# gabrielmittag/NISQA

Measured on AMD Instinct MI355X. Metric: clips/sec (10 s, 48 kHz), higher is better.
Workload: dtype bf16x6 (every GEMM -- CNN, projection, self-attention, pooling: fp32 operands as three exact bf16 terms, 6 MFMA products per term pair, f32 accumulate: all 24 operand mantissa bits; mel f32)

## Files before the change

nisqa_amd/csrc/cnn_bf16.hip:

```cpp
#include "common.hpp"
#include "layout.hpp"
#include <stdlib.h>
#include <atomic>
#include "conv_bf16.hpp"
#include "internal.hpp"
#include "../../include/nisqa_hip.h"
#define NQ_RING2 3
#define NQ_RING34 3

#define FB_RS1 48
#define FB_P1 (168 * FB_RS1)
#define FB_RS2 80
#define FB_P2 (60 * FB_RS2)
#define FB_RS3 144
#define FB_P3 (60 * FB_RS3)
#define FB_PS (72 * FB_RS3)
#define FB_PATCH(T) ((T) * FB_P1)
#define FB_PPLANE 1700
#define FB_ZADDR 2048u
#define FB_BASE 2176u
#define FB_WAVE(T) (((T) * (FB_P1 + FB_PPLANE) + 63u) / 64u * 64u)
#define FB_WGS(T) ((T) == 2 ? 2 : 1)
#define FB_LDS(T) (FB_BASE + 4 * FB_WAVE(T))
static_assert(FB_WAVE(2) == 19584 && FB_LDS(2) == 80512 && 2 * FB_LDS(2) <= 160 * 1024, "two terms: two workgroups (8 waves) per CU");
static_assert(FB_WAVE(3) == 29312 && FB_LDS(3) == 119424 && FB_LDS(3) <= 160 * 1024 && 2 * FB_LDS(3) > 160 * 1024, "three terms: one workgroup per CU");
#define FB_PLAN_OK(T) (FB_PATCH(T) + (T) * FB_PPLANE <= FB_WAVE(T) && (T) * FB_P3 <= FB_WAVE(T) && (T) * FB_PS <= 2 * FB_WAVE(T))
static_assert(FB_PLAN_OK(2) && FB_PLAN_OK(3), "LDS plan");

__device__ constexpr int bwin75_lo(int b) { return b == 0 ? 0 : b == 1 ? 1 : b == 2 ? 2 : b == 3 ? 4 : 5; }
__device__ constexpr int bwin75_hi(int b) { return b == 0 ? 2 : b == 1 ? 3 : b == 2 ? 5 : b == 3 ? 6 : 7; }
__device__ constexpr int bwin53_lo(int b) { return b == 0 ? 0 : b == 1 ? 1 : 3; }
__device__ constexpr int bwin53_hi(int b) { return b == 0 ? 2 : b == 1 ? 4 : 5; }

NQ_CLK_EXPORT(g_phase_clk, nisqa_debug_phase_clock)
NQ_CLK_EXPORT(g_phase_clk6, nisqa_debug_phase_clock6)

#define FB_TAB5 0u
#define FB_TAB6 1024u
NQ_DEV f32x2_t lds_ld64(unsigned a) { return *(NQ_AS3 const f32x2_t*)(a); }
template <int FMT>
NQ_DEV float epi_fmt(float v, float c, float t) {
    return FMT == NQ_FMT_BF16X3 || FMT == NQ_FMT_BF16X6 ? fmaxf(v + t, 0.f) : fmaxf(fmaf(v, c, t), 0.f);
}

template <int FMT, int CIN, int MT, int NT, int W, int RS, int PLANE, bool APF, int RING>
NQ_DEV void fb_conv_k(f32x16 (&acc)[MT][NT], __amdgpu_buffer_rsrc_t wrs, int wbyte, unsigned lane16, const unsigned (&base)[MT],
                      const unsigned (&m9)[MT], conv_k_ring<FMT == NQ_FMT_BF16X6 ? 3 : 2, NT, 3>& ring) {
    if constexpr (FMT == NQ_FMT_BF16X6) conv_k_terms_ring<3, CIN, MT, NT, W, RS, PLANE, FB_ZADDR, 3, true, true>(acc, wrs, wbyte, lane16, base, m9, ring);
    else conv_k_bf16<CIN, MT, NT, W, RS, PLANE, FB_ZADDR, APF, RING, FMT>(acc, wrs, wbyte, lane16, base, m9);
}

template <int FMT, bool SEGX, bool P3>
NQ_DEV void cnn_front_split_body(
    const float* __restrict__ mel_tm, const int32_t* __restrict__ frame_off,
    const int32_t* __restrict__ tok_off, const int32_t* __restrict__ n_wins,
    const float* __restrict__ clip_floor, int n_clips, int seg_hop,
    const float* __restrict__ cw, const unsigned short* __restrict__ wb, float* __restrict__ p3,
    float* __restrict__ feat, const float* __restrict__ seg_x, int seg_L,
    const uint32_t* __restrict__ clip_max_enc, float top_db) {
    extern __shared__ __attribute__((aligned(16))) char smem[];
    constexpr bool X6 = FMT == NQ_FMT_BF16X6, F16 = FMT == NQ_FMT_F16X3 || FMT == NQ_FMT_F16X4;
    constexpr int T = X6 ? 3 : 2;
    constexpr bool T16_3 = X6 && (NQ_T16 & 1), T16_4 = X6 && (NQ_T16 & 2);
    static_assert(!P3 || FMT == NQ_FMT_BF16X3, "the fp32 copy of the pooled conv4 tensor is a bf16x3 debug output");
    constexpr int W1_ = X6 ? CNNX_W1 : CNNB_W1, W2_ = X6 ? CNNX_W2 : CNNB_W2, W3_ = X6 ? CNNX_W3 : CNNB_W3, W4_ = X6 ? CNNX_W4 : CNNB_W4,
                  W5_ = X6 ? CNNX_W5 : CNNB_W5, W6_ = X6 ? CNNX_W6 : CNNB_W6, WU16_ = X6 ? CNNX_U16S : CNNB_U16S;
    const int* __restrict__ meta_i = (const int*)(wb + CNNH_META);
    const float* __restrict__ meta_f = (const float*)(wb + CNNH_META);
    float dummy_mx = 0.f;
    NQ_STAMP_BEGIN();
    const int lane = threadIdx.x & 63;
    const int wave = __builtin_amdgcn_readfirstlane(threadIdx.x >> 6);
    const int p0 = blockIdx.x * 4;
    const int b = __builtin_amdgcn_readfirstlane(find_segment_wave(tok_off, n_clips, p0, lane));
    const int k0 = p0 - tok_off[b];
    const int nvalid = min(4, n_wins[b] - k0);
    if (nvalid <= 0) return;
    const bool valid = wave < nvalid;
    const int p = p0 + wave, k = k0 + wave;
    const unsigned R = FB_BASE + wave * FB_WAVE(T);
    const unsigned lane16 = lane * 16;
    const __amdgpu_buffer_rsrc_t wrs = __builtin_amdgcn_make_buffer_rsrc((void*)wb, 0, WU16_ * 2, 0x00020000);
    NQ_STAMP(0);

    const float fl = SEGX ? -3.0e38f : clip_max_enc ? dec_ordered(clip_max_enc[b]) - top_db : clip_floor[b];
    const float* src = SEGX ? seg_x + ((size_t)b * seg_L + k) * 720
                            : mel_tm + (size_t)(frame_off[b] + k * seg_hop) * 48;
    float vraw[12];
#pragma unroll
    for (int q = 0; q < 12; ++q) {
        const int i0 = lane + 64 * q;
        vraw[q] = (valid && (q < 11 || lane < 16)) ? src[i0] : 0.f;
    }
    const float tn1 = cw[CNN_T1 + (lane & 15)], tn2 = cw[CNN_T2 + (lane & 31)];
    const float tn3[2] = {cw[CNN_T3 + (lane & 31)], cw[CNN_T3 + 32 + (lane & 31)]};
    const float tn4[2] = {cw[CNN_T4 + (lane & 31)], cw[CNN_T4 + 32 + (lane & 31)]};
    const float tn5 = cw[CNN_T5 + 16 * wave + (lane & 15)], tn6 = cw[CNN_T6 + 16 * wave + (lane & 15)];
    float vin[12];
#pragma unroll
    for (int q = 0; q < 12; ++q) vin[q] = !valid ? 0.f : SEGX ? vraw[q] : fmaxf(vraw[q], fl);
    int e_in = 0;
    float m_in = 0.f;
    float s0 = 1.f;
    if (F16) {
        float mr = 0.f;
#pragma unroll
        for (int q = 0; q < 12; ++q) mr = fmaxf(mr, __builtin_fabsf(vin[q]));
        m_in = wave_max_nonneg(mr);
        e_in = f16_scale_exp(m_in);
        s0 = pow2_f32(e_in);
    }
    {
        const unsigned pb = R + FB_PATCH(T);
        constexpr int NZ = (T * FB_PPLANE + 15) / 16;
#pragma unroll
        for (int it = 0; it < (NZ + 63) / 64; ++it)
            if (64 * it + 64 <= NZ || lane < NZ - 64 * it) lds_st128(pb + (lane + 64 * it) * 16, f32x4{0.f, 0.f, 0.f, 0.f});
        if (lane < 32) ((unsigned*)(smem + FB_ZADDR))[lane] = 0u;
        __builtin_amdgcn_wave_barrier();
        if (!SEGX) {
            unsigned ob[3];
#pragma unroll
            for (int u = 0; u < 3; ++u) {
                const int e = lane + 16 * u, j0 = e >= 48 ? 1 : 0, m = e - 48 * j0;
                ob[u] = pb + ((j0 + 1) * 50 + m + 1) * 2;
            }
#pragma unroll
            for (int q = 0; q < 12; q += 2) {
                const float v0 = vin[q] * s0, v1 = vin[q + 1] * s0;
                lds_store_pair_fmt<FMT>(ob[q % 3] + (q + q / 3) * 100, ob[(q + 1) % 3] + (q + 1 + (q + 1) / 3) * 100, FB_PPLANE, v0, v1,
                                               dummy_mx, true, q + 1 < 11 || lane < 16);
            }
        } else {
#pragma unroll
            for (int q = 0; q < 12; ++q) {
                const int i0 = lane + 64 * q;
                const int m = i0 / 15, j = i0 - 15 * m;
                if (i0 < 720) lds_store_one_fmt<FMT>(pb + ((j + 1) * 50 + (m + 1)) * 2, FB_PPLANE, vin[q] * s0, dummy_mx);
            }
        }
    }
    __builtin_amdgcn_wave_barrier();
    NQ_STAMP(1);

    const int i = lane & 31, hfi = (i >> 2) & 1, qi = (i & 3) + 4 * (i >> 3);
    const int n = lane & 31, hf = lane >> 5, h = lane >> 5;

    conv_k_ring<T, 1, 3> ring2;
    if constexpr (X6) conv_k_preload(ring2, wrs, W2_ * 2, lane16);
    {
        f32x4 w1[1][T];
#pragma unroll
        for (int t = 0; t < T; ++t) w1[0][t] = wfrag_load(wrs, lane16, (W1_ + t * 512) * 2);
        float tn = tn1, c1 = 1.f, ms1 = 0.f;
        int e1 = 0;
        if (F16) {
            e1 = f16_scale_exp(fmaf(m_in, meta_f[8], meta_f[16]));
            c1 = pow2_f32(e1 - e_in - meta_i[0]);
            tn = tn1 * pow2_f32(e1);
        }
        const int xq = min(qi, 14);
        unsigned rd_a = R + FB_PATCH(T) + ((xq + (h ? 2 : 0)) * 50 + 24 * hfi) * 2;
        unsigned rd_b = R + FB_PATCH(T) + ((xq + (h ? 2 : 1)) * 50 + 24 * hfi) * 2;
        const bool is_b = (n & 16) != 0;
        const unsigned mb = is_b ? ~0u : 0u;
        unsigned wr = R + (12 * hf * 7) * FB_RS1 + (n & 15) * 2 + (is_b ? FB_RS1 : 0);
        for (int g2 = 0; g2 < 6; ++g2) {
            f32x16 acc[2][1];
            f32x4 xa[2][T];
#pragma unroll
            for (int tt = 0; tt < 2; ++tt)
#pragma unroll
                for (int t = 0; t < T; ++t) {
                    const unsigned pa = rd_a + 4 * tt + t * FB_PPLANE, pq = rd_b + 4 * tt + t * FB_PPLANE;
                    xa[tt][t] = f32x4{__uint_as_float(lds_ld32(pa)), __uint_as_float(lds_ld32(pa + 4)),
                                      __uint_as_float(lds_ld32(pq)), __uint_as_float(lds_ld32(pq + 4))};
                }
            acc[0][0] = zero16();
            acc[1][0] = zero16();
            if constexpr (X6) {
                mma_terms<T, 2, 1>(acc, xa, w1);
            } else {
                const f32x4 (&w)[T] = w1[0];
                if (FMT == NQ_FMT_F16X4) { acc[0][0] = mfma32_fmt<FMT>(xa[0][1], w[1], acc[0][0]); acc[1][0] = mfma32_fmt<FMT>(xa[1][1], w[1], acc[1][0]); }
                acc[0][0] = mfma32_fmt<FMT>(xa[0][1], w[0], acc[0][0]); acc[1][0] = mfma32_fmt<FMT>(xa[1][1], w[0], acc[1][0]);
                acc[0][0] = mfma32_fmt<FMT>(xa[0][0], w[1], acc[0][0]); acc[1][0] = mfma32_fmt<FMT>(xa[1][0], w[1], acc[1][0]);
                acc[0][0] = mfma32_fmt<FMT>(xa[0][0], w[0], acc[0][0]); acc[1][0] = mfma32_fmt<FMT>(xa[1][0], w[0], acc[1][0]);
            }
            unsigned r[14];
#pragma unroll
            for (int v = 0; v < 14; ++v) {
                const int tt = v / 7, bb = v - 7 * tt;
                const float mx = fmaxf(fmaxf(acc[tt][0][2 * bb], acc[tt][0][2 * bb + 1]), acc[tt][0][2 * bb + 2]);
                r[v] = __float_as_uint(epi_fmt<FMT>(mx, c1, tn));
            }
            unsigned got[7];
#pragma unroll
            for (int kk = 0; kk < 7; ++kk)
                got[kk] = (unsigned)__builtin_amdgcn_ds_swizzle((int)((r[2 * kk] & mb) | (r[2 * kk + 1] & ~mb)), 0x401F);
            float fin[7];
#pragma unroll
            for (int kk = 0; kk < 7; ++kk) {
                const unsigned own = (r[2 * kk + 1] & mb) | (r[2 * kk] & ~mb);
                fin[kk] = __uint_as_float(max(own, got[kk]));
            }
#pragma unroll
            for (int kk = 0; kk < 6; kk += 2) lds_store_pair_fmt<FMT>(wr + 2 * kk * FB_RS1, wr + 2 * (kk + 1) * FB_RS1, FB_P1, fin[kk], fin[kk + 1], ms1);
            lds_store_one_fmt<FMT>(wr + 12 * FB_RS1, FB_P1, fin[6], ms1);
            rd_a += 8; rd_b += 8;
            wr += 14 * FB_RS1;
        }
        if (F16) { m_in = wave_max_nonneg(ms1) * pow2_f32(-e1); e_in = e1; }
    }

    NQ_STAMP(2);
    conv_k_ring<T, 2, 3> ring34;
    conv_kt_ring<T, 4, NQ_RINGT> ringt;
    const unsigned lanew = conv_kt_lane<T, 4>(lane);
    const int c16 = lane & 15, q4 = lane >> 4;
    f32x4 tnt[4];
    {
        f32x16 acc[6][1];
        unsigned base[6], m9[6];
#pragma unroll
        for (int t = 0; t < 6; ++t) {
            acc[t][0] = zero16();
            const int u = 16 * t + qi;
            const int gl = u / 14, w = u % 14, yy = w / 7;
            const int py = 2 * (6 * hfi + gl) + yy, px = w - 7 * yy;
            m9[t] = tap_mask(u < 84, py, px, 24, 7);
            base[t] = R + ((py - 1) * 7 + (px - 1)) * FB_RS1 + (h << 4);
        }
        fb_conv_k<FMT, 16, 6, 1, 7, FB_RS1, FB_P1, false, NQ_RING2>(acc, wrs, W2_ * 2, lane16, base, m9, ring2);
        NQ_STAMP(3);
        if constexpr (T16_3) {
            conv_kt_preload(ringt, wrs, W3_ * 2, lanew);
#pragma unroll
            for (int mt = 0; mt < 4; ++mt) tnt[mt] = *(const f32x4*)(cw + CNN_T3 + 16 * mt + 4 * q4);
            __builtin_amdgcn_sched_barrier(0);
        } else if constexpr (X6) {
            conv_k_preload(ring34, wrs, W3_ * 2, lane16);
            __builtin_amdgcn_sched_barrier(0);
        }
        float tn = tn2, c2 = 1.f, ms2 = 0.f;
        int e2 = 0;
        if (F16) {
            e2 = f16_scale_exp(fmaf(m_in, meta_f[9], meta_f[17]));
            c2 = pow2_f32(e2 - e_in - meta_i[1]);
            tn = tn2 * pow2_f32(e2);
        }
        const unsigned wr = R + (6 * hf * 5) * FB_RS2 + n * 2;
#pragma unroll
        for (int k2 = 0; k2 < 30; k2 += 2) {
            float pv[2];
#pragma unroll
            for (int e = 0; e < 2; ++e) {
                const int gl = (k2 + e) / 5, bb = (k2 + e) % 5;
                float mx = -3.0e38f;
#pragma unroll
                for (int yy = 0; yy < 2; ++yy)
#pragma unroll
                    for (int x = bwin75_lo(bb); x < bwin75_hi(bb); ++x) {
                        const int u = 14 * gl + 7 * yy + x;
                        mx = fmaxf(mx, acc[u >> 4][0][u & 15]);
                    }
                pv[e] = epi_fmt<FMT>(mx, c2, tn);
            }
            lds_store_pair_fmt<FMT>(wr + k2 * FB_RS2, wr + (k2 + 1) * FB_RS2, FB_P2, pv[0], pv[1], ms2);
        }
        if (F16) { m_in = wave_max_nonneg(ms2) * pow2_f32(-e2); e_in = e2; }
    }

    NQ_STAMP(4);
    unsigned base34[2], m34[2];
#pragma unroll
    for (int t = 0; t < 2; ++t) {
        const int u = 16 * t + qi;
        const int gl = u / 10, w = u % 10, yy = w / 5;
        const int py = 2 * (3 * hfi + gl) + yy, px = w - 5 * yy;
        m34[t] = tap_mask(u < 30, py, px, 12, 5);
        base34[t] = (py - 1) * 5 + (px - 1);
    }

    if constexpr (T16_3) {
        f32x4 acc[4][4];
        unsigned base[4], m9[4];
#pragma unroll
        for (int nt = 0; nt < 4; ++nt) {
#pragma unroll
            for (int mt = 0; mt < 4; ++mt) acc[mt][nt] = f32x4{0.f, 0.f, 0.f, 0.f};
            const int pix = 16 * nt + c16, py = pix / 5, px = pix - 5 * py;
            m9[nt] = tap_mask(pix < 60, py, px, 12, 5);
            base[nt] = R + (pix - 6) * FB_RS2 + (q4 << 4);
        }
        conv_kt_terms_ring<3, 32, 4, 4, 5, FB_RS2, FB_P2, FB_ZADDR, NQ_RINGT>(acc, wrs, W3_ * 2, lanew, base, m9, ringt);
        NQ_STAMP(5);
        const f32x4 tn[4] = {tnt[0], tnt[1], tnt[2], tnt[3]};
        if constexpr (T16_4) {
            conv_kt_preload(ringt, wrs, W4_ * 2, lanew);
#pragma unroll
            for (int mt = 0; mt < 4; ++mt) tnt[mt] = *(const f32x4*)(cw + CNN_T4 + 16 * mt + 4 * q4);
        } else conv_k_preload(ring34, wrs, W4_ * 2, lane16);
        __builtin_amdgcn_sched_barrier(0);
        const unsigned wr = R + c16 * FB_RS3 + q4 * 8;
#pragma unroll
        for (int nt = 0; nt < 4; ++nt)
            if (nt < 3 || c16 < 12) {
#pragma unroll
                for (int mt = 0; mt < 4; ++mt) {
                    f32x4 v;
#pragma unroll
                    for (int r = 0; r < 4; ++r) v[r] = fmaxf(acc[mt][nt][r] + tn[mt][r], 0.f);
                    lds_store_terms4<3>(wr + 16 * nt * FB_RS3 + 32 * mt, FB_P3, v);
                }
            }
    } else {
        f32x16 acc[2][2];
        unsigned base[2];
#pragma unroll
        for (int t = 0; t < 2; ++t) {
#pragma unroll
            for (int nt = 0; nt < 2; ++nt) acc[t][nt] = zero16();
            base[t] = R + base34[t] * FB_RS2 + (h << 4);
        }
        fb_conv_k<FMT, 32, 2, 2, 5, FB_RS2, FB_P2, true, NQ_RING34>(acc, wrs, W3_ * 2, lane16, base, m34, ring34);
        NQ_STAMP(5);
        if constexpr (T16_4) {
            conv_kt_preload(ringt, wrs, W4_ * 2, lanew);
#pragma unroll
            for (int mt = 0; mt < 4; ++mt) tnt[mt] = *(const f32x4*)(cw + CNN_T4 + 16 * mt + 4 * q4);
            __builtin_amdgcn_sched_barrier(0);
        } else if constexpr (X6) {
            conv_k_preload(ring34, wrs, W4_ * 2, lane16);
            __builtin_amdgcn_sched_barrier(0);
        }
        float tn[2] = {tn3[0], tn3[1]}, c3 = 1.f, ms3 = 0.f;
        int e3 = 0;
        if (F16) {
            e3 = f16_scale_exp(fmaf(m_in, meta_f[10], meta_f[18]));
            c3 = pow2_f32(e3 - e_in - meta_i[2]);
            tn[0] *= pow2_f32(e3);
            tn[1] *= pow2_f32(e3);
        }
        const unsigned wr = R + (6 * hf * 5) * FB_RS3 + n * 2;
#pragma unroll
        for (int nt = 0; nt < 2; ++nt)
#pragma unroll
            for (int t = 0; t < 2; ++t)
#pragma unroll
                for (int r = 0; r < 16; r += 2) {
                    const int u = 16 * t + r;
                    if (u < 30)
                        lds_store_pair_fmt<FMT>(wr + u * FB_RS3 + 64 * nt, wr + (u + 1) * FB_RS3 + 64 * nt, FB_P3,
                                                epi_fmt<FMT>(acc[t][nt][r], c3, tn[nt]), epi_fmt<FMT>(acc[t][nt][r + 1], c3, tn[nt]), ms3);
                }
        if (F16) { m_in = wave_max_nonneg(ms3) * pow2_f32(-e3); e_in = e3; }
    }

    NQ_STAMP(6);
    const unsigned S4 = FB_BASE;
    const unsigned S5 = FB_BASE + 2 * FB_WAVE(T);
    const int w5b = __builtin_amdgcn_readfirstlane((W5_ + wave * (18 * T * 512)) * 2);
    const int w6b = __builtin_amdgcn_readfirstlane((W6_ + wave * (18 * T * 512)) * 2);
    f32x4 b5[4][T], b6[8][T];
    if constexpr (T16_4) {
        f32x4 acc[4][4];
        unsigned base[4], m9[4];
        const int j5 = c16 / 5, role = c16 - 5 * j5;
        const int glc = 2 * j5 + (role >= 3 ? 1 : 0);
#pragma unroll
        for (int nt = 0; nt < 4; ++nt) {
#pragma unroll
            for (int mt = 0; mt < 4; ++mt) acc[mt][nt] = f32x4{0.f, 0.f, 0.f, 0.f};
            const int yy = nt & 1, hi = nt >> 1;
            const int gl = role == 2 ? 2 * j5 + hi : glc;
            const int px = role == 2 ? 2 : role == 0 ? hi : role == 3 ? 1 - hi : 3 + hi, py = 2 * gl + yy;
            m9[nt] = tap_mask(c16 < 15, py, px, 12, 5);
            base[nt] = R + (py * 5 + px - 6) * FB_RS3 + (q4 << 4);
        }
        conv_kt_terms_ring<3, 64, 4, 4, 5, FB_RS3, FB_P3, FB_ZADDR, NQ_RINGT>(acc, wrs, W4_ * 2, lanew, base, m9, ringt);
        NQ_STAMP(7);
#pragma unroll
        for (int g = 0; g < 3; ++g)
#pragma unroll
            for (int q = 0; q < T; ++q) b5[g][q] = wfrag_load(wrs, lane16, w5b + (g * T + q) * 1024);
        f32x4 w02[4], w1[4];
#pragma unroll
        for (int mt = 0; mt < 4; ++mt)
#pragma unroll
            for (int r = 0; r < 4; ++r) {
                const float m01 = __builtin_elementwise_maximum(acc[mt][0][r], acc[mt][1][r]), m23 = __builtin_elementwise_maximum(acc[mt][2][r], acc[mt][3][r]);
                const int i01 = (int)__float_as_uint(m01), i23 = (int)__float_as_uint(m23);
                const float lf = __uint_as_float((unsigned)__builtin_amdgcn_update_dpp(i23, i23, 0x111, 0xf, 0xf, false));
                const float rt = __uint_as_float((unsigned)__builtin_amdgcn_update_dpp(i01, i01, 0x101, 0xf, 0xf, false));
                w02[mt][r] = fmaxf(__builtin_elementwise_maximum(m01, m23) + tnt[mt][r], 0.f);
                w1[mt][r] = fmaxf(__builtin_elementwise_maximum(__builtin_elementwise_maximum(m01, lf), rt) + tnt[mt][r], 0.f);
            }
        __syncthreads();
        const unsigned wr = S4 + (18 * wave + 3 * glc) * FB_RS3 + q4 * 8;
        if (c16 < 15 && role != 2) {
            const unsigned a = wr + (role == 1 || role == 4 ? 2 * FB_RS3 : 0);
#pragma unroll
            for (int mt = 0; mt < 4; ++mt) lds_store_terms4<3>(a + 32 * mt, FB_PS, w02[mt]);
        }
        if (c16 < 15 && (role == 1 || role == 3)) {
#pragma unroll
            for (int mt = 0; mt < 4; ++mt) lds_store_terms4<3>(wr + FB_RS3 + 32 * mt, FB_PS, w1[mt]);
        }
    } else {
        f32x16 acc[2][2];
        unsigned base[2];
#pragma unroll
        for (int t = 0; t < 2; ++t) {
#pragma unroll
            for (int nt = 0; nt < 2; ++nt) acc[t][nt] = zero16();
            base[t] = R + base34[t] * FB_RS3 + (h << 4);
        }
        fb_conv_k<FMT, 64, 2, 2, 5, FB_RS3, FB_P3, true, NQ_RING34>(acc, wrs, W4_ * 2, lane16, base, m34, ring34);
        NQ_STAMP(7);
        float tn[2] = {tn4[0], tn4[1]}, c4 = 1.f, ms4 = 0.f;
        int e4 = 0;
        if (F16) {
            e4 = f16_scale_exp(fmaf(m_in, meta_f[11], meta_f[19]));
            c4 = pow2_f32(e4 - e_in - meta_i[3]);
            tn[0] *= pow2_f32(e4);
            tn[1] *= pow2_f32(e4);
        }
#pragma unroll
        for (int g = 0; g < 3; ++g)
#pragma unroll
            for (int q = 0; q < T; ++q) b5[g][q] = wfrag_load(wrs, lane16, w5b + (g * T + q) * 1024);
        __syncthreads();
        const unsigned wr = S4 + (18 * wave + 9 * hf) * FB_RS3 + n * 2;
        float* dst = P3 ? p3 + (size_t)p * (18 * 64) : nullptr;
#pragma unroll
        for (int gl = 0; gl < 3; ++gl)
#pragma unroll
            for (int bb = 0; bb < 3; ++bb) {
                float pv[2];
#pragma unroll
                for (int nt = 0; nt < 2; ++nt) {
                    float mx = -3.0e38f;
#pragma unroll
                    for (int yy = 0; yy < 2; ++yy)
#pragma unroll
                        for (int x = bwin53_lo(bb); x < bwin53_hi(bb); ++x) {
                            const int u = 10 * gl + 5 * yy + x;
                            mx = fmaxf(mx, acc[u >> 4][nt][u & 15]);
                        }
                    pv[nt] = epi_fmt<FMT>(mx, c4, tn[nt]);
                    if (P3 && valid) dst[((3 * hf + gl) * 3 + bb) * 64 + n + 32 * nt] = pv[nt];
                }
                lds_store_pair_fmt<FMT>(wr + (gl * 3 + bb) * FB_RS3, wr + (gl * 3 + bb) * FB_RS3 + 64, FB_PS, pv[0], pv[1], ms4);
            }
        if (F16) {
            const float m4 = wave_max_nonneg(ms4) * pow2_f32(-e4);
            const int e5 = f16_scale_exp(fmaf(m4, meta_f[12], meta_f[20]));
            if (lane < 18) {
                lds_st32(FB_TAB5 + (18 * wave + lane) * 8, __float_as_uint(pow2_f32(e5 - e4 - meta_i[4])));
                lds_st32(FB_TAB5 + (18 * wave + lane) * 8 + 4, __float_as_uint(pow2_f32(e5)));
            }
            if (lane < 6) lds_st32(FB_TAB6 + (6 * wave + lane) * 4, __float_as_uint(pow2_f32(-(e5 + meta_i[5]))));
        }
    }
    __syncthreads();
    NQ_STAMP(8);

    {
        const int i16 = lane & 15, kg = lane >> 4;
        const int ch = 16 * wave + i16;
        f32x4 acc5[5];
        unsigned base5[5], m5[5];
#pragma unroll
        for (int t = 0; t < 5; ++t) {
            acc5[t] = f32x4{0.f, 0.f, 0.f, 0.f};
            const int rho = 16 * t + i16;
            const int slot = rho / 18, pix = rho - 18 * slot, ry = pix / 3, rx = pix - 3 * ry;
            m5[t] = tap_mask(rho < 72, ry, rx, 6, 3);
            base5[t] = S4 + (slot * 18 + (ry - 1) * 3 + (rx - 1)) * FB_RS3 + (kg << 4);
        }
        unsigned a5ad[5][T];
        f32x4 a5[2][5][T];
        auto load_a5 = [&](int g) {
            const int tap = g >> 1, s = g & 1;
            const int tapoff = ((tap / 3) * 3 + tap % 3) * FB_RS3;
            if (s == 0) {
#pragma unroll
                for (int t = 0; t < 5; ++t) {
                    const bool ok = (m5[t] >> tap) & 1u;
#pragma unroll
                    for (int q = 0; q < T; ++q) a5ad[t][q] = ok ? base5[t] + q * FB_PS : FB_ZADDR - tapoff;
                }
            }
#pragma unroll
            for (int t = 0; t < 5; ++t)
#pragma unroll
                for (int q = 0; q < T; ++q) a5[g & 1][t][q] = lds_ld128(a5ad[t][q] + tapoff + 64 * s);
        };
        load_a5(0);
#pragma unroll
        for (int g = 0; g < 18; ++g) {
            if (g + 3 < 18) {
#pragma unroll
                for (int q = 0; q < T; ++q) b5[(g + 3) & 3][q] = wfrag_load(wrs, lane16, w5b + ((g + 3) * T + q) * 1024);
            }
            if (g + 1 < 18) load_a5(g + 1);
            if constexpr (X6) {
                __builtin_amdgcn_sched_barrier(0);
                mma16_terms<T, 5>(acc5, a5[g & 1], b5[g & 3]);
            } else mma16_pair_fmt<FMT, 5>(acc5, a5[g & 1], b5[g & 3]);
        }
        NQ_STAMP(9);
#pragma unroll
        for (int g = 0; g < 7; ++g)
#pragma unroll
            for (int q = 0; q < T; ++q) b6[g][q] = wfrag_load(wrs, lane16, w6b + (g * T + q) * 1024);
        {
            const unsigned wr = S5 + (4 * kg) * FB_RS3 + ch * 2;
#pragma unroll
            for (int t = 0; t < 5; ++t)
#pragma unroll
                for (int r = 0; r < 4; r += 2)
                    if (t < 4 || kg < 2) {
                        f32x2_t cs0 = {1.f, 1.f}, cs1 = {1.f, 1.f};
                        if (F16) { cs0 = lds_ld64(FB_TAB5 + (16 * t + r) * 8 + kg * 32); cs1 = lds_ld64(FB_TAB5 + (16 * t + r + 1) * 8 + kg * 32); }
                        lds_store_pair_fmt<FMT>(wr + (16 * t + r) * FB_RS3, wr + (16 * t + r + 1) * FB_RS3, FB_PS,
                                                epi_fmt<FMT>(acc5[t][r], cs0[0], tn5 * cs0[1]), epi_fmt<FMT>(acc5[t][r + 1], cs1[0], tn5 * cs1[1]), dummy_mx);
                    }
        }
        __syncthreads();
        NQ_STAMP(10);

        f32x4 acc6[2], acc6b[2];
        unsigned base6[2], m6[2];
#pragma unroll
        for (int t = 0; t < 2; ++t) {
            acc6[t] = f32x4{0.f, 0.f, 0.f, 0.f};
            acc6b[t] = acc6[t];
            const int rho = 16 * t + i16;
            const int slot = rho / 6, y = rho - 6 * slot;
            m6[t] = tap_mask(rho < 24, y, 1, 6, 3);
            base6[t] = S5 + (slot * 18 + (y - 1) * 3) * FB_RS3 + (kg << 4);
        }
        unsigned a6ad[2][T];
        f32x4 a6[2][2][T];
        auto load_a6 = [&](int g) {
            const int tap = g >> 1, s = g & 1;
            const int tapoff = ((tap / 3) * 3 + tap % 3) * FB_RS3;
            if (s == 0) {
#pragma unroll
                for (int t = 0; t < 2; ++t) {
                    const bool ok = (m6[t] >> tap) & 1u;
#pragma unroll
                    for (int q = 0; q < T; ++q) a6ad[t][q] = ok ? base6[t] + q * FB_PS : FB_ZADDR - tapoff;
                }
            }
#pragma unroll
            for (int t = 0; t < 2; ++t)
#pragma unroll
                for (int q = 0; q < T; ++q) a6[g & 1][t][q] = lds_ld128(a6ad[t][q] + tapoff + 64 * s);
        };
        load_a6(0);
#pragma unroll
        for (int g = 0; g < 18; ++g) {
            if (g + 7 < 18) {
#pragma unroll
                for (int q = 0; q < T; ++q) b6[(g + 7) & 7][q] = wfrag_load(wrs, lane16, w6b + ((g + 7) * T + q) * 1024);
            }
            if (g + 1 < 18) load_a6(g + 1);
            f32x4 (&acc)[2] = (g & 1) ? acc6b : acc6;
            if constexpr (X6) {
// ... 140 lines not shown
```

nisqa_amd/csrc/conv_bf16.hpp:

```cpp
#pragma once
#include "bf16_terms.hpp"

#define NQ_FMT_BF16X3 0
#define NQ_FMT_F16X3 1
#define NQ_FMT_F16X4 2
#define NQ_FMT_BF16X6 3
typedef _Float16 f16x8 __attribute__((ext_vector_type(8)));
typedef _Float16 f16x2_t __attribute__((ext_vector_type(2)));
template <int FMT>
NQ_DEV f32x16 mfma32_fmt(f32x4 a, f32x4 b, f32x16 c) {
    if (FMT == NQ_FMT_BF16X3) return mfma_bf(a, b, c);
    return __builtin_amdgcn_mfma_f32_32x32x16_f16(__builtin_bit_cast(f16x8, a), __builtin_bit_cast(f16x8, b), c, 0, 0, 0);
}
template <int FMT>
NQ_DEV f32x4 mfma16_fmt(f32x4 a, f32x4 b, f32x4 c) {
    if (FMT == NQ_FMT_BF16X3) return mfma_bf16x16(a, b, c);
    return __builtin_amdgcn_mfma_f32_16x16x32_f16(__builtin_bit_cast(f16x8, a), __builtin_bit_cast(f16x8, b), c, 0, 0, 0);
}
template <int FMT, int MT, int NT>
NQ_DEV void mma_pair_fmt(f32x16 (&acc)[MT][NT], const f32x4 (&ah)[MT], const f32x4 (&al)[MT], const f32x4 (&bh)[NT], const f32x4 (&bl)[NT]) {
    if (FMT == NQ_FMT_F16X4) {
#pragma unroll
        for (int t = 0; t < MT; ++t)
#pragma unroll
            for (int nt = 0; nt < NT; ++nt) acc[t][nt] = mfma32_fmt<FMT>(al[t], bl[nt], acc[t][nt]);
    }
#pragma unroll
    for (int t = 0; t < MT; ++t)
#pragma unroll
        for (int nt = 0; nt < NT; ++nt) acc[t][nt] = mfma32_fmt<FMT>(ah[t], bl[nt], acc[t][nt]);
#pragma unroll
    for (int t = 0; t < MT; ++t)
#pragma unroll
        for (int nt = 0; nt < NT; ++nt) acc[t][nt] = mfma32_fmt<FMT>(al[t], bh[nt], acc[t][nt]);
#pragma unroll
    for (int t = 0; t < MT; ++t)
#pragma unroll
        for (int nt = 0; nt < NT; ++nt) acc[t][nt] = mfma32_fmt<FMT>(ah[t], bh[nt], acc[t][nt]);
}
template <int FMT, int MT>
NQ_DEV void mma16_pair_fmt(f32x4 (&acc)[MT], const f32x4 (&a)[MT][2], const f32x4 (&b)[2]) {
    if (FMT == NQ_FMT_F16X4) {
#pragma unroll
        for (int t = 0; t < MT; ++t) acc[t] = mfma16_fmt<FMT>(a[t][1], b[1], acc[t]);
    }
#pragma unroll
    for (int t = 0; t < MT; ++t) acc[t] = mfma16_fmt<FMT>(a[t][0], b[1], acc[t]);
#pragma unroll
    for (int t = 0; t < MT; ++t) acc[t] = mfma16_fmt<FMT>(a[t][1], b[0], acc[t]);
#pragma unroll
    for (int t = 0; t < MT; ++t) acc[t] = mfma16_fmt<FMT>(a[t][0], b[0], acc[t]);
}
NQ_DEV int f16_scale_exp(float bound) {
    const int be = (int)((__float_as_uint(bound) >> 23) & 0xffu);
    return min(max(15 - (be - 126), -60), 60);
}
NQ_DEV float pow2_f32(int e) { return __uint_as_float((unsigned)(min(max(e, -126), 127) + 127) << 23); }
NQ_DEV float wave_max_nonneg(float v) {
    int x = (int)__float_as_uint(v);
    x = max(x, __builtin_amdgcn_update_dpp(x, x, 0xB1, 0xf, 0xf, false));
    x = max(x, __builtin_amdgcn_update_dpp(x, x, 0x4E, 0xf, 0xf, false));
    x = max(x, __builtin_amdgcn_update_dpp(x, x, 0x141, 0xf, 0xf, false));
    x = max(x, __builtin_amdgcn_update_dpp(x, x, 0x140, 0xf, 0xf, false));
    const unsigned m = max(max((unsigned)__builtin_amdgcn_readlane(x, 0), (unsigned)__builtin_amdgcn_readlane(x, 16)),
                           max((unsigned)__builtin_amdgcn_readlane(x, 32), (unsigned)__builtin_amdgcn_readlane(x, 48)));
    return __uint_as_float(m);
}

NQ_DEV unsigned bf16_bits(float v) {
    const unsigned u = __float_as_uint(v);
    return (u + 0x7fffu + ((u >> 16) & 1u)) >> 16;
}
NQ_DEV float bf16_val(unsigned b) { return __uint_as_float(b << 16); }

NQ_DEV void store_split(char* plane_hi, int plane_bytes, int off, float v) {
    const unsigned hi = cvt_pk_bf16(v, 0.f);
    const unsigned lo = cvt_pk_bf16(v - __uint_as_float(hi << 16), 0.f);
    *(unsigned short*)(plane_hi + off) = (unsigned short)hi;
    *(unsigned short*)(plane_hi + plane_bytes + off) = (unsigned short)lo;
}

#ifndef NQ_SB
#define NQ_SB 0
#endif
#define NQ_STEP_FENCE() do { if (NQ_SB & 1) __builtin_amdgcn_sched_barrier(0); } while (0)
#define NQ_ISSUE_FENCE() do { if (NQ_SB & 2) __builtin_amdgcn_sched_barrier(0); } while (0)
NQ_DEV f32x4 lds_ld128(unsigned a) { return *(NQ_AS3 const f32x4*)(a); }
NQ_DEV unsigned lds_ld32(unsigned a) { return *(NQ_AS3 const unsigned*)(a); }
NQ_DEV void lds_st16(unsigned a, unsigned v) { *(NQ_AS3 unsigned short*)(a) = (unsigned short)v; }
NQ_DEV void lds_st32(unsigned a, unsigned v) { *(NQ_AS3 unsigned*)(a) = v; }
NQ_DEV void lds_st64(unsigned a, u32x2 v) { *(NQ_AS3 u32x2*)(a) = v; }
NQ_DEV void lds_st128(unsigned a, f32x4 v) { *(NQ_AS3 f32x4*)(a) = v; }
NQ_DEV void lds_store_split(unsigned a, int plane, float v) {
    const unsigned hi = cvt_pk_bf16(v, 0.f);
    const unsigned lo = cvt_pk_bf16(v - __uint_as_float(hi << 16), 0.f);
    lds_st16(a, hi);
    lds_st16(a + plane, lo);
}
NQ_DEV void lds_st16_hi(unsigned a, unsigned v) { *(NQ_AS3 unsigned short*)(a) = (unsigned short)(v >> 16); }
NQ_DEV void lds_store_split2(unsigned a0, unsigned a1, int plane, float v0, float v1, bool st0 = true, bool st1 = true) {
    const unsigned hi2 = cvt_pk_bf16(v0, v1);
    const f32x2_t vv = {v0, v1};
    const f32x2_t hf = {__uint_as_float(hi2 << 16), __uint_as_float(hi2 & 0xffff0000u)};
    const f32x2_t r = vv - hf;
    const unsigned lo2 = cvt_pk_bf16(r[0], r[1]);
    if (st0) { lds_st16(a0, hi2); lds_st16(a0 + plane, lo2); }
    if (st1) { lds_st16_hi(a1, hi2); lds_st16_hi(a1 + plane, lo2); }
}
NQ_DEV unsigned cvt_pk_f16(float a, float b) {
    const f32x2_t v = {a, b};
    return __builtin_bit_cast(unsigned, __builtin_convertvector(v, f16x2_t));
}
template <int T> NQ_DEV void lds_store_terms2(unsigned a0, unsigned a1, int plane, float v0, float v1, bool st0 = true, bool st1 = true);
template <int T> NQ_DEV void lds_store_terms(unsigned a, int plane, float v);
template <int FMT>
NQ_DEV void lds_store_pair_fmt(unsigned a0, unsigned a1, int plane, float v0, float v1, float& mx, bool st0 = true, bool st1 = true) {
    if (FMT == NQ_FMT_BF16X3) { lds_store_split2(a0, a1, plane, v0, v1, st0, st1); return; }
    if (FMT == NQ_FMT_BF16X6) { lds_store_terms2<3>(a0, a1, plane, v0, v1, st0, st1); return; }
    const unsigned hi2 = cvt_pk_f16(v0, v1);
    const f32x2_t vv = {v0, v1};
    const f32x2_t hf = __builtin_convertvector(__builtin_bit_cast(f16x2_t, hi2), f32x2_t);
    const f32x2_t r = vv - hf;
    const unsigned lo2 = cvt_pk_f16(r[0], r[1]);
    mx = fmaxf(fmaxf(mx, __builtin_fabsf(v0)), __builtin_fabsf(v1));
    if (st0) { lds_st16(a0, hi2); lds_st16(a0 + plane, lo2); }
    if (st1) { lds_st16_hi(a1, hi2); lds_st16_hi(a1 + plane, lo2); }
}
template <int FMT>
NQ_DEV void lds_store_one_fmt(unsigned a, int plane, float v, float& mx) {
    if (FMT == NQ_FMT_BF16X3) { lds_store_split(a, plane, v); return; }
    if (FMT == NQ_FMT_BF16X6) { lds_store_terms<3>(a, plane, v); return; }
    const unsigned hi = cvt_pk_f16(v, 0.f);
    const float hf = (float)__builtin_bit_cast(f16x2_t, hi)[0];
    const unsigned lo = cvt_pk_f16(v - hf, 0.f);
    mx = fmaxf(mx, __builtin_fabsf(v));
    lds_st16(a, hi);
    lds_st16(a + plane, lo);
}
NQ_DEV f32x16 splat16(float v) { f32x16 r; for (int q = 0; q < 16; ++q) r[q] = v; return r; }
typedef int nq_i32x4 __attribute__((ext_vector_type(4)));
NQ_DEV f32x4 wfrag_load(__amdgpu_buffer_rsrc_t rsrc, unsigned lane16, int byte_off) {
    return __builtin_bit_cast(f32x4, __builtin_amdgcn_raw_buffer_load_b128(rsrc, lane16, byte_off, 0));
}
NQ_DEV unsigned tap_mask(bool valid, int y, int x, int H, int W) {
    unsigned m = 0;
#pragma unroll
    for (int tap = 0; tap < 9; ++tap) {
        const int yy = y + tap / 3 - 1, xx = x + tap % 3 - 1;
        m |= (valid && (unsigned)yy < (unsigned)H && (unsigned)xx < (unsigned)W) ? (1u << tap) : 0u;
    }
    return m;
}

template <int CIN, int MT, int NT, int W, int RS, int PLANE, unsigned ZADDR, bool APF, int RING = 3, int FMT = NQ_FMT_BF16X3>
NQ_DEV void conv_k_bf16(f32x16 (&acc)[MT][NT], __amdgpu_buffer_rsrc_t rsrc, int wbyte, unsigned lane16,
                        const unsigned (&base)[MT], const unsigned (&m9)[MT]) {
    constexpr int S16 = CIN / 16, TOTAL = 9 * S16, AB = APF ? 2 : 1;
    static_assert(ZADDR >= (2 * W + 2) * RS + 32 * S16, "zero block must sit above the largest tap offset");
    f32x4 bh[RING][NT], bl[RING][NT], ah[AB][MT], al[AB][MT];
    unsigned a_hi[MT], a_lo[MT];
    auto load_b = [&](int g, int slot) {
#pragma unroll
        for (int nt = 0; nt < NT; ++nt) {
            bh[slot][nt] = wfrag_load(rsrc, lane16, wbyte + ((g * NT + nt) * 2 + 0) * 1024);
            bl[slot][nt] = wfrag_load(rsrc, lane16, wbyte + ((g * NT + nt) * 2 + 1) * 1024);
        }
    };
    auto load_a = [&](int g, int slot) {
        const int tap = g / S16, s = g - tap * S16;
        const int tapoff = ((tap / 3) * W + tap % 3) * RS;
        if (s == 0) {
#pragma unroll
            for (int t = 0; t < MT; ++t) {
                const bool ok = (m9[t] >> tap) & 1u;
                a_hi[t] = ok ? base[t] : ZADDR - tapoff;
                a_lo[t] = ok ? base[t] + PLANE : ZADDR - tapoff;
            }
        }
#pragma unroll
        for (int t = 0; t < MT; ++t) {
            ah[slot][t] = lds_ld128(a_hi[t] + tapoff + 32 * s);
            al[slot][t] = lds_ld128(a_lo[t] + tapoff + 32 * s);
        }
    };
#pragma unroll
    for (int g = 0; g < RING - 1; ++g) load_b(g, g);
    if (APF) load_a(0, 0);
#pragma unroll
    for (int g = 0; g < TOTAL; ++g) {
        NQ_STEP_FENCE();
        if (g + RING - 1 < TOTAL) load_b(g + RING - 1, (g + RING - 1) % RING);
        if (APF) { if (g + 1 < TOTAL) load_a(g + 1, (g + 1) & 1); } else load_a(g, 0);
        NQ_ISSUE_FENCE();
        const int sa = APF ? (g & 1) : 0, sb = g % RING;
        mma_pair_fmt<FMT, MT, NT>(acc, ah[sa], al[sa], bh[sb], bl[sb]);
    }
}


template <int T>
NQ_DEV void lds_store_terms2(unsigned a0, unsigned a1, int plane, float v0, float v1, bool st0, bool st1) {
    f32x2_t r = {v0, v1};
#pragma unroll
    for (int t = 0; t < T; ++t) {
        const unsigned pk = cvt_pk_bf16(r[0], r[1]);
        if (st0) lds_st16(a0 + t * plane, pk);
        if (st1) lds_st16_hi(a1 + t * plane, pk);
        if (t + 1 < T) {
            const f32x2_t part = {__uint_as_float(pk << 16), __uint_as_float(pk & 0xffff0000u)};
            r = r - part;
        }
    }
}
template <int T>
NQ_DEV void lds_store_terms(unsigned a, int plane, float v) {
    float r = v;
#pragma unroll
    for (int t = 0; t < T; ++t) {
        const unsigned pk = cvt_pk_bf16(r, 0.f);
        lds_st16(a + t * plane, pk);
        if (t + 1 < T) r -= __uint_as_float(pk << 16);
    }
}
template <int T>
NQ_DEV void lds_store_terms4(unsigned a, int plane, f32x4 v) {
    unsigned lo[T], hi[T];
    split2t<T>(v[0], v[1], lo);
    split2t<T>(v[2], v[3], hi);
#pragma unroll
    for (int t = 0; t < T; ++t) lds_st64(a + t * plane, u32x2{lo[t], hi[t]});
}
template <int T, int NT, int RING = 3>
struct conv_k_ring { f32x4 b[RING][NT][T]; };
template <int T, int NT, int RING>
NQ_DEV void conv_k_preload(conv_k_ring<T, NT, RING>& r, __amdgpu_buffer_rsrc_t rsrc, int wbyte, unsigned lane16) {
#pragma unroll
    for (int g = 0; g < RING - 1; ++g)
#pragma unroll
        for (int nt = 0; nt < NT; ++nt)
#pragma unroll
            for (int t = 0; t < T; ++t) r.b[g][nt][t] = wfrag_load(rsrc, lane16, wbyte + ((g * NT + nt) * T + t) * 1024);
}
template <int T, int CIN, int MT, int NT, int W, int RS, int PLANE, unsigned ZADDR, int RING, bool FENCE, bool PRE>
NQ_DEV void conv_k_terms_ring(f32x16 (&acc)[MT][NT], __amdgpu_buffer_rsrc_t rsrc, int wbyte, unsigned lane16,
                              const unsigned (&base)[MT], const unsigned (&m9)[MT], conv_k_ring<T, NT, RING>& ring) {
    constexpr int S16 = CIN / 16, TOTAL = 9 * S16;
    static_assert(ZADDR >= (2 * W + 2) * RS + 32 * S16, "zero block must sit above the largest tap offset");
    f32x4 a[2][MT][T];
    unsigned a_ad[MT][T];
    auto load_b = [&](int g, int slot) {
#pragma unroll
        for (int nt = 0; nt < NT; ++nt)
#pragma unroll
            for (int t = 0; t < T; ++t) ring.b[slot][nt][t] = wfrag_load(rsrc, lane16, wbyte + ((g * NT + nt) * T + t) * 1024);
    };
    auto load_a = [&](int g, int slot) {
        const int tap = g / S16, s = g - tap * S16;
        const int tapoff = ((tap / 3) * W + tap % 3) * RS;
        if (s == 0) {
#pragma unroll
            for (int m = 0; m < MT; ++m) {
                const bool ok = (m9[m] >> tap) & 1u;
#pragma unroll
                for (int t = 0; t < T; ++t) a_ad[m][t] = ok ? base[m] + t * PLANE : ZADDR - tapoff;
            }
        }
#pragma unroll
        for (int m = 0; m < MT; ++m)
#pragma unroll
            for (int t = 0; t < T; ++t) a[slot][m][t] = lds_ld128(a_ad[m][t] + tapoff + 32 * s);
    };
    if (!PRE) {
#pragma unroll
        for (int g = 0; g < RING - 1; ++g) load_b(g, g);
    }
    load_a(0, 0);
#pragma unroll
    for (int g = 0; g < TOTAL; ++g) {
        if (g + RING - 1 < TOTAL) load_b(g + RING - 1, (g + RING - 1) % RING);
        if (g + 1 < TOTAL) load_a(g + 1, (g + 1) & 1);
        if (FENCE) __builtin_amdgcn_sched_barrier(0);
        mma_terms<T, MT, NT>(acc, a[g & 1], ring.b[g % RING]);
    }
}
#ifndef NQ_KT_SGB
#define NQ_KT_SGB 1
#endif
#ifndef NQ_T16
#define NQ_T16 3
#endif
#ifndef NQ_RINGT
#define NQ_RINGT 2
#endif
template <int T, int MT, int RING = 3>
struct conv_kt_ring { f32x4 a[RING][MT][T]; };
template <int T, int MT>
NQ_DEV unsigned conv_kt_lane(int lane) {
    const int q = lane >> 4;
    return (unsigned)((q >> 1) * ((MT / 2) * T * 1024) + ((lane & 15) + 32 * (q & 1)) * 16);
}
template <int T, int MT>
NQ_DEV f32x4 conv_kt_wfrag(__amdgpu_buffer_rsrc_t rsrc, unsigned lanew, int wbyte, int G, int mt, int t) {
    return wfrag_load(rsrc, lanew, wbyte + ((2 * G * (MT / 2) + (mt >> 1)) * T + t) * 1024 + (mt & 1) * 256);
}
template <int T, int MT, int RING>
NQ_DEV void conv_kt_preload(conv_kt_ring<T, MT, RING>& r, __amdgpu_buffer_rsrc_t rsrc, int wbyte, unsigned lanew) {
#pragma unroll
    for (int G = 0; G < RING - 1; ++G)
#pragma unroll
        for (int mt = 0; mt < MT; ++mt)
#pragma unroll
            for (int t = 0; t < T; ++t) r.a[G][mt][t] = conv_kt_wfrag<T, MT>(rsrc, lanew, wbyte, G, mt, t);
}
template <int T, int CIN, int MT, int NT, int W, int RS, int PLANE, unsigned ZADDR, int RING>
NQ_DEV void conv_kt_terms_ring(f32x4 (&acc)[MT][NT], __amdgpu_buffer_rsrc_t rsrc, int wbyte, unsigned lanew,
                               const unsigned (&base)[NT], const unsigned (&m9)[NT], conv_kt_ring<T, MT, RING>& ring) {
    constexpr int S32 = CIN / 32, TOTAL = 9 * S32;
    static_assert(MT % 2 == 0 && CIN % 32 == 0, "whole 32-channel fragment tiles");
    static_assert(ZADDR >= (2 * W + 2) * RS + 64 * S32, "zero block must sit above the largest tap offset");
    f32x4 b[2][NT][T];
    unsigned b_ad[NT][T];
    auto load_a = [&](int G, int slot) {
#pragma unroll
        for (int mt = 0; mt < MT; ++mt)
#pragma unroll
            for (int t = 0; t < T; ++t) ring.a[slot][mt][t] = conv_kt_wfrag<T, MT>(rsrc, lanew, wbyte, G, mt, t);
    };
    auto load_b = [&](int G, int slot) {
        const int tap = G / S32, s = G - tap * S32;
        const int tapoff = ((tap / 3) * W + tap % 3) * RS;
        if (s == 0) {
#pragma unroll
            for (int nt = 0; nt < NT; ++nt) {
                const bool ok = (m9[nt] >> tap) & 1u;
#pragma unroll
                for (int t = 0; t < T; ++t) b_ad[nt][t] = ok ? base[nt] + t * PLANE : ZADDR - tapoff;
            }
        }
#pragma unroll
        for (int nt = 0; nt < NT; ++nt)
#pragma unroll
            for (int t = 0; t < T; ++t) b[slot][nt][t] = lds_ld128(b_ad[nt][t] + tapoff + 64 * s);
    };
    load_b(0, 0);
#pragma unroll
    for (int G = 0; G < TOTAL; ++G) {
#if NQ_KT_SGB
        __builtin_amdgcn_sched_barrier(0);
        mma16_terms<T, MT, NT>(acc, ring.a[G % RING], b[G & 1]);
        if (G + RING - 1 < TOTAL) load_a(G + RING - 1, (G + RING - 1) % RING);
        if (G + 1 < TOTAL) load_b(G + 1, (G + 1) & 1);
#pragma unroll
        for (int i = 0; i < MT * T; ++i) {
            __builtin_amdgcn_sched_group_barrier(0x008, 2, 0);
            __builtin_amdgcn_sched_group_barrier(0x002, 2, 0);
            __builtin_amdgcn_sched_group_barrier(0x008, 2, 0);
            __builtin_amdgcn_sched_group_barrier(0x100, 1, 0);
            __builtin_amdgcn_sched_group_barrier(0x008, 2, 0);
            __builtin_amdgcn_sched_group_barrier(0x020, 1, 0);
            __builtin_amdgcn_sched_group_barrier(0x008, MT * NT * T * (T + 1) / 2 / (MT * T) - 6, 0);
        }
#else
        if (G + RING - 1 < TOTAL) load_a(G + RING - 1, (G + RING - 1) % RING);
        if (G + 1 < TOTAL) load_b(G + 1, (G + 1) & 1);
        __builtin_amdgcn_sched_barrier(0);
        mma16_terms<T, MT, NT>(acc, ring.a[G % RING], b[G & 1]);
#endif
    }
}
template <int T, int CIN, int MT, int NT, int W, int RS, int PLANE, unsigned ZADDR, int RING = 3, bool FENCE = true>
NQ_DEV void conv_k_terms(f32x16 (&acc)[MT][NT], __amdgpu_buffer_rsrc_t rsrc, int wbyte, unsigned lane16,
                         const unsigned (&base)[MT], const unsigned (&m9)[MT]) {
    conv_k_ring<T, NT, RING> ring;
    conv_k_terms_ring<T, CIN, MT, NT, W, RS, PLANE, ZADDR, RING, FENCE, false>(acc, rsrc, wbyte, lane16, base, m9, ring);
}
```

Baseline: 62980.

## Pair channel stores via DPP and software-pipeline conv1 MFMA with pooling

Adds a cross-lane store path in which adjacent lanes swap values through DPP, so each lane writes one 32-bit word holding a channel pair per bf16 term instead of two 16-bit stores. This is used for the conv1 and conv2 outputs in the bf16x6 path. Conv1 is also software-pipelined: the MFMA for the next group is issued while the current group is pooled, with sched_group_barrier interleaving MFMAs and VALU ops. The gain is fewer LDS store instructions and better overlap of the MFMA and VALU units, at the cost of extra DPP operations and more live accumulator registers.

```diff
diff --git a/nisqa_amd/csrc/cnn_bf16.hip b/nisqa_amd/csrc/cnn_bf16.hip
--- a/nisqa_amd/csrc/cnn_bf16.hip
+++ b/nisqa_amd/csrc/cnn_bf16.hip
@@ -62,6 +62,7 @@
     constexpr bool X6 = FMT == NQ_FMT_BF16X6, F16 = FMT == NQ_FMT_F16X3 || FMT == NQ_FMT_F16X4;
     constexpr int T = X6 ? 3 : 2;
     constexpr bool T16_3 = X6 && (NQ_T16 & 1), T16_4 = X6 && (NQ_T16 & 2);
+    constexpr bool CP1 = X6 && (NQ_CPAIR & 1), CP2 = X6 && (NQ_CPAIR & 2);
     static_assert(!P3 || FMT == NQ_FMT_BF16X3, "the fp32 copy of the pooled conv4 tensor is a bf16x3 debug output");
     constexpr int W1_ = X6 ? CNNX_W1 : CNNB_W1, W2_ = X6 ? CNNX_W2 : CNNB_W2, W3_ = X6 ? CNNX_W3 : CNNB_W3, W4_ = X6 ? CNNX_W4 : CNNB_W4,
                   W5_ = X6 ? CNNX_W5 : CNNB_W5, W6_ = X6 ? CNNX_W6 : CNNB_W6, WU16_ = X6 ? CNNX_U16S : CNNB_U16S;
@@ -145,6 +146,7 @@
 
     const int i = lane & 31, hfi = (i >> 2) & 1, qi = (i & 3) + 4 * (i >> 3);
     const int n = lane & 31, hf = lane >> 5, h = lane >> 5;
+    const bool odd = (lane & 1) != 0;
 
     conv_k_ring<T, 1, 3> ring2;
     if constexpr (X6) conv_k_preload(ring2, wrs, W2_ * 2, lane16);
@@ -165,14 +167,16 @@
         const bool is_b = (n & 16) != 0;
         const unsigned mb = is_b ? ~0u : 0u;
         unsigned wr = R + (12 * hf * 7) * FB_RS1 + (n & 15) * 2 + (is_b ? FB_RS1 : 0);
-        for (int g2 = 0; g2 < 6; ++g2) {
-            f32x16 acc[2][1];
+        const unsigned wrc = R + (12 * hf * 7) * FB_RS1 + (n & 14) * 2 + (is_b ? FB_RS1 : 0);
+        const unsigned wrp = wrc + (odd ? 2 * FB_RS1 : 0), wrq = wrc + (odd ? 14 * FB_RS1 : 0);
+        float fin6 = 0.f;
+        auto c1_mma = [&](f32x16 (&acc)[2][1], unsigned ra, unsigned rb) {
             f32x4 xa[2][T];
 #pragma unroll
             for (int tt = 0; tt < 2; ++tt)
 #pragma unroll
                 for (int t = 0; t < T; ++t) {
-                    const unsigned pa = rd_a + 4 * tt + t * FB_PPLANE, pq = rd_b + 4 * tt + t * FB_PPLANE;
+                    const unsigned pa = ra + 4 * tt + t * FB_PPLANE, pq = rb + 4 * tt + t * FB_PPLANE;
                     xa[tt][t] = f32x4{__uint_as_float(lds_ld32(pa)), __uint_as_float(lds_ld32(pa + 4)),
                                       __uint_as_float(lds_ld32(pq)), __uint_as_float(lds_ld32(pq + 4))};
                 }
@@ -187,6 +191,8 @@
                 acc[0][0] = mfma32_fmt<FMT>(xa[0][0], w[1], acc[0][0]); acc[1][0] = mfma32_fmt<FMT>(xa[1][0], w[1], acc[1][0]);
                 acc[0][0] = mfma32_fmt<FMT>(xa[0][0], w[0], acc[0][0]); acc[1][0] = mfma32_fmt<FMT>(xa[1][0], w[0], acc[1][0]);
             }
+        };
+        auto c1_pool = [&](const f32x16 (&acc)[2][1], unsigned w, int g2) {
             unsigned r[14];
 #pragma unroll
             for (int v = 0; v < 14; ++v) {
@@ -204,11 +210,42 @@
                 const unsigned own = (r[2 * kk + 1] & mb) | (r[2 * kk] & ~mb);
                 fin[kk] = __uint_as_float(max(own, got[kk]));
             }
-#pragma unroll
-            for (int kk = 0; kk < 6; kk += 2) lds_store_pair_fmt<FMT>(wr + 2 * kk * FB_RS1, wr + 2 * (kk + 1) * FB_RS1, FB_P1, fin[kk], fin[kk + 1], ms1);
-            lds_store_one_fmt<FMT>(wr + 12 * FB_RS1, FB_P1, fin[6], ms1);
-            rd_a += 8; rd_b += 8;
-            wr += 14 * FB_RS1;
+            if constexpr (CP1) {
+#pragma unroll
+                for (int kk = 0; kk < 6; kk += 2) lds_store_terms2_cpair<T>(wrp + (14 * g2 + 2 * kk) * FB_RS1, FB_P1, fin[kk], fin[kk + 1], odd);
+                if (g2 & 1) lds_store_terms2_cpair<T>(wrq + (14 * (g2 - 1) + 12) * FB_RS1, FB_P1, fin6, fin[6], odd);
+                else fin6 = fin[6];
+            } else {
+#pragma unroll
+                for (int kk = 0; kk < 6; kk += 2) lds_store_pair_fmt<FMT>(w + 2 * kk * FB_RS1, w + 2 * (kk + 1) * FB_RS1, FB_P1, fin[kk], fin[kk + 1], ms1);
+                lds_store_one_fmt<FMT>(w + 12 * FB_RS1, FB_P1, fin[6], ms1);
+            }
+        };
+        if constexpr (X6 && NQ_C1_PIPE) {
+            f32x16 acc[2][2][1];
+            c1_mma(acc[0], rd_a, rd_b);
+#pragma unroll
+            for (int g2 = 0; g2 < 6; ++g2) {
+                __builtin_amdgcn_sched_barrier(0);
+                if (g2 + 1 < 6) c1_mma(acc[(g2 + 1) & 1], rd_a + 8 * (g2 + 1), rd_b + 8 * (g2 + 1));
+                c1_pool(acc[g2 & 1], wr + 14 * g2 * FB_RS1, g2);
+                if (g2 + 1 < 6) {
+#pragma unroll
+                    for (int i = 0; i < 12; ++i) {
+                        __builtin_amdgcn_sched_group_barrier(0x008, 1, 0);
+                        __builtin_amdgcn_sched_group_barrier(0x002, NQ_C1_PIPE, 0);
+                    }
+                }
+            }
+        } else {
+#pragma unroll
+            for (int g2 = 0; g2 < 6; ++g2) {
+                f32x16 acc[2][1];
+                c1_mma(acc, rd_a, rd_b);
+                c1_pool(acc, wr, g2);
+                rd_a += 8; rd_b += 8;
+                wr += 14 * FB_RS1;
+            }
         }
         if (F16) { m_in = wave_max_nonneg(ms1) * pow2_f32(-e1); e_in = e1; }
     }
@@ -250,6 +287,7 @@
             tn = tn2 * pow2_f32(e2);
         }
         const unsigned wr = R + (6 * hf * 5) * FB_RS2 + n * 2;
+        const unsigned wrp = R + (6 * hf * 5) * FB_RS2 + (n & 30) * 2 + (odd ? FB_RS2 : 0);
 #pragma unroll
         for (int k2 = 0; k2 < 30; k2 += 2) {
             float pv[2];
@@ -266,7 +304,8 @@
                     }
                 pv[e] = epi_fmt<FMT>(mx, c2, tn);
             }
-            lds_store_pair_fmt<FMT>(wr + k2 * FB_RS2, wr + (k2 + 1) * FB_RS2, FB_P2, pv[0], pv[1], ms2);
+            if constexpr (CP2) lds_store_terms2_cpair<T>(wrp + k2 * FB_RS2, FB_P2, pv[0], pv[1], odd);
+            else lds_store_pair_fmt<FMT>(wr + k2 * FB_RS2, wr + (k2 + 1) * FB_RS2, FB_P2, pv[0], pv[1], ms2);
         }
         if (F16) { m_in = wave_max_nonneg(ms2) * pow2_f32(-e2); e_in = e2; }
     }
diff --git a/nisqa_amd/csrc/conv_bf16.hpp b/nisqa_amd/csrc/conv_bf16.hpp
--- a/nisqa_amd/csrc/conv_bf16.hpp
+++ b/nisqa_amd/csrc/conv_bf16.hpp
@@ -230,6 +230,22 @@
 #pragma unroll
     for (int t = 0; t < T; ++t) lds_st64(a + t * plane, u32x2{lo[t], hi[t]});
 }
+#ifndef NQ_CPAIR
+#define NQ_CPAIR 3
+#endif
+#ifndef NQ_C1_PIPE
+#define NQ_C1_PIPE 8
+#endif
+template <int T>
+NQ_DEV void lds_store_terms2_cpair(unsigned a, int plane, float v0, float v1, bool odd) {
+    const int i0 = (int)__float_as_uint(v0), i1 = (int)__float_as_uint(v1);
+    const float g0 = __uint_as_float((unsigned)__builtin_amdgcn_update_dpp(0, i0, 0xB1, 0xf, 0xf, true));
+    const float g1 = __uint_as_float((unsigned)__builtin_amdgcn_update_dpp(0, i1, 0xB1, 0xf, 0xf, true));
+    unsigned t[T];
+    split2t<T>(odd ? g1 : v0, odd ? v1 : g0, t);
+#pragma unroll
+    for (int q = 0; q < T; ++q) lds_st32(a + q * plane, t[q]);
+}
 template <int T, int NT, int RING = 3>
 struct conv_k_ring { f32x4 b[RING][NT][T]; };
 template <int T, int NT, int RING>
```

Result: faster. 63630, median of 6 (+1.0%).
